# spacemeshos/go-spacemesh

Hardware: AMD Instinct MI355X
Metric: post_labels_per_sec (higher is better)
Workload: dtype u32; 1 GPU; init-mainnet-scryptN8192-4units-256GiB-sink; step_labels=2097152, scrypt_n=8192, num_units=4, labels_per_unit=4294967296, parallelism=index-range shards x1, RCCL nonce min-reduce, vrf_nonce_found=True

## Files before the change

go-spacemesh_amd/csrc/kernels.hip:

```cpp
#include <hip/hip_runtime.h>

#include <cstdlib>
#include <cstring>

#include "kernel_args.h"
#include "post_common.h"

#define POSTE_THREADS 256

#if defined(POSTE_NT) && POSTE_NT
typedef uint32_t poste_v4u __attribute__((ext_vector_type(4)));
#define VSTORE(p, v)                                                           \
  do {                                                                         \
    uint4 _t = (v);                                                            \
    __builtin_nontemporal_store(*(poste_v4u *)&_t, (poste_v4u *)(p));          \
  } while (0)
#define VLOAD(p)                                                               \
  ({                                                                           \
    poste_v4u _r = __builtin_nontemporal_load((const poste_v4u *)(p));         \
    *(uint4 *)&_r;                                                             \
  })
#else
#define VSTORE(p, v) (*(p) = (v))
#define VLOAD(p) (*(p))
#endif

__constant__ uint32_t c_sha_k[64] = {
    0x428a2f98, 0x71374491, 0xb5c0fbcf, 0xe9b5dba5, 0x3956c25b, 0x59f111f1,
    0x923f82a4, 0xab1c5ed5, 0xd807aa98, 0x12835b01, 0x243185be, 0x550c7dc3,
    0x72be5d74, 0x80deb1fe, 0x9bdc06a7, 0xc19bf174, 0xe49b69c1, 0xefbe4786,
    0x0fc19dc6, 0x240ca1cc, 0x2de92c6f, 0x4a7484aa, 0x5cb0a9dc, 0x76f988da,
    0x983e5152, 0xa831c66d, 0xb00327c8, 0xbf597fc7, 0xc6e00bf3, 0xd5a79147,
    0x06ca6351, 0x14292967, 0x27b70a85, 0x2e1b2138, 0x4d2c6dfc, 0x53380d13,
    0x650a7354, 0x766a0abb, 0x81c2c92e, 0x92722c85, 0xa2bfe8a1, 0xa81a664b,
    0xc24b8b70, 0xc76c51a3, 0xd192e819, 0xd6990624, 0xf40e3585, 0x106aa070,
    0x19a4c116, 0x1e376c08, 0x2748774c, 0x34b0bcb5, 0x391c0cb3, 0x4ed8aa4a,
    0x5b9cca4f, 0x682e6ff3, 0x748f82ee, 0x78a5636f, 0x84c87814, 0x8cc70208,
    0x90befffa, 0xa4506ceb, 0xbef9a3f7, 0xc67178f2};

__device__ __forceinline__ uint32_t ror32(uint32_t x, int n) {
  return __builtin_rotateright32(x, n);
}

__device__ void sha_compress(uint32_t h[8], const uint32_t m[16]) {
  uint32_t w[16];
#pragma unroll
  for (int i = 0; i < 16; i++) w[i] = m[i];
  uint32_t a = h[0], b = h[1], c = h[2], d = h[3];
  uint32_t e = h[4], f = h[5], g = h[6], hh = h[7];
#pragma unroll
  for (int t = 0; t < 64; t++) {
    uint32_t wt;
    if (t < 16) {
      wt = w[t];
    } else {
      uint32_t a15 = w[(t - 15) & 15], a2 = w[(t - 2) & 15];
      wt = w[t & 15] += (ror32(a15, 7) ^ ror32(a15, 18) ^ (a15 >> 3)) +
                        w[(t - 7) & 15] +
                        (ror32(a2, 17) ^ ror32(a2, 19) ^ (a2 >> 10));
    }
    uint32_t t1 = hh + (ror32(e, 6) ^ ror32(e, 11) ^ ror32(e, 25)) +
                  ((e & f) ^ (~e & g)) + c_sha_k[t] + wt;
    uint32_t t2 = (ror32(a, 2) ^ ror32(a, 13) ^ ror32(a, 22)) +
                  ((a & b) ^ (a & c) ^ (b & c));
    hh = g; g = f; f = e; e = d + t1;
    d = c; c = b; b = a; a = t1 + t2;
  }
  h[0] += a; h[1] += b; h[2] += c; h[3] += d;
  h[4] += e; h[5] += f; h[6] += g; h[7] += hh;
}

__device__ __forceinline__ void sha_init(uint32_t h[8]) {
  h[0] = 0x6a09e667; h[1] = 0xbb67ae85; h[2] = 0x3c6ef372; h[3] = 0xa54ff53a;
  h[4] = 0x510e527f; h[5] = 0x9b05688c; h[6] = 0x1f83d9ab; h[7] = 0x5be0cd19;
}


#define SWZ(v, pat)                                                            \
  ((uint32_t)__builtin_amdgcn_mov_dpp((int)(v), (pat), 0xf, 0xf, true))
#define QROT1 0x39
#define QROT2 0x4E
#define QROT3 0x93
#define QBCAST0 0x00

__device__ __forceinline__ void salsa8_z(uint32_t &A, uint32_t &B,
                                         uint32_t &C, uint32_t &D) {
  uint32_t a = A, b = B, c = C, d = D;
#pragma unroll
  for (int i = 0; i < 4; i++) {
    b ^= __builtin_rotateleft32(a + d, 7);
    c ^= __builtin_rotateleft32(b + a, 9);
    d ^= __builtin_rotateleft32(c + b, 13);
    a ^= __builtin_rotateleft32(d + c, 18);
    uint32_t y1 = SWZ(d, QROT1);
    uint32_t y2 = SWZ(c, QROT2);
    uint32_t y3 = SWZ(b, QROT3);
    y1 ^= __builtin_rotateleft32(a + y3, 7);
    y2 ^= __builtin_rotateleft32(y1 + a, 9);
    y3 ^= __builtin_rotateleft32(y2 + y1, 13);
    a ^= __builtin_rotateleft32(y3 + y2, 18);
    d = SWZ(y1, QROT3);
    c = SWZ(y2, QROT2);
    b = SWZ(y3, QROT1);
  }
  A += a; B += b; C += c; D += d;
}

__device__ __forceinline__ void blockmix_z(uint32_t X0[4], uint32_t X1[4]) {
  uint32_t t0 = X0[0] ^ X1[0], t1 = X0[1] ^ X1[1], t2 = X0[2] ^ X1[2],
           t3 = X0[3] ^ X1[3];
  salsa8_z(t0, t1, t2, t3);
  X0[0] = t0; X0[1] = t1; X0[2] = t2; X0[3] = t3;
  t0 ^= X1[0]; t1 ^= X1[1]; t2 ^= X1[2]; t3 ^= X1[3];
  salsa8_z(t0, t1, t2, t3);
  X1[0] = t0; X1[1] = t1; X1[2] = t2; X1[3] = t3;
}

__device__ __forceinline__ void canon_to_z(const uint32_t x[16], uint32_t sub,
                                           uint32_t z[4]) {
  uint32_t s0 = sub == 0 ? x[0] : sub == 1 ? x[5] : sub == 2 ? x[10] : x[15];
  uint32_t s1 = sub == 0 ? x[4] : sub == 1 ? x[9] : sub == 2 ? x[14] : x[3];
  uint32_t s2 = sub == 0 ? x[8] : sub == 1 ? x[13] : sub == 2 ? x[2] : x[7];
  uint32_t s3 = sub == 0 ? x[12] : sub == 1 ? x[1] : sub == 2 ? x[6] : x[11];
  z[0] = s0; z[1] = s1; z[2] = s2; z[3] = s3;
}

__device__ __forceinline__ void z_to_msg_be(const uint32_t z[4],
                                            uint32_t m[16]) {
#pragma unroll
  for (int v = 0; v < 4; v++) {
    m[(4 * v + 0) & 15] = __builtin_bswap32(SWZ(z[v], 0x00));
    m[(4 * v + 5) & 15] = __builtin_bswap32(SWZ(z[v], 0x55));
    m[(4 * v + 10) & 15] = __builtin_bswap32(SWZ(z[v], 0xAA));
    m[(4 * v + 15) & 15] = __builtin_bswap32(SWZ(z[v], 0xFF));
  }
}


__device__ __forceinline__ void hmac_outer(const uint32_t ho[8],
                                           const uint32_t inner[8],
                                           uint32_t out[8]) {
  uint32_t h[8], m[16];
#pragma unroll
  for (int i = 0; i < 8; i++) h[i] = ho[i];
#pragma unroll
  for (int i = 0; i < 8; i++) m[i] = inner[i];
  m[8] = 0x80000000u;
#pragma unroll
  for (int i = 9; i < 15; i++) m[i] = 0;
  m[15] = (64 + 32) * 8;
  sha_compress(h, m);
#pragma unroll
  for (int i = 0; i < 8; i++) out[i] = h[i];
}


__device__ __forceinline__ void hmac_states_for(const uint32_t *cw,
                                                unsigned long long index,
                                                uint32_t hi[8],
                                                uint32_t ho[8]) {
  uint32_t pw_be[10], m[16];
#pragma unroll
  for (int i = 0; i < 8; i++) pw_be[i] = __builtin_bswap32(cw[i]);
  pw_be[8] = __builtin_bswap32((uint32_t)index);
  pw_be[9] = __builtin_bswap32((uint32_t)(index >> 32));
  sha_init(hi);
#pragma unroll
  for (int i = 0; i < 10; i++) m[i] = pw_be[i] ^ 0x36363636u;
#pragma unroll
  for (int i = 10; i < 16; i++) m[i] = 0x36363636u;
  sha_compress(hi, m);
  sha_init(ho);
#pragma unroll
  for (int i = 0; i < 10; i++) m[i] = pw_be[i] ^ 0x5c5c5c5cu;
#pragma unroll
  for (int i = 10; i < 16; i++) m[i] = 0x5c5c5c5cu;
  sha_compress(ho, m);
}

__global__ void __launch_bounds__(POSTE_THREADS)
post_label_prologue_kernel(LabelKernelArgs a) {
  const unsigned long long lane =
      (unsigned long long)blockIdx.x * blockDim.x + threadIdx.x;
  const unsigned long long group = lane >> 2;
  const unsigned long long gstride =
      ((unsigned long long)gridDim.x * blockDim.x) >> 2;
  const uint32_t sub = (uint32_t)(lane & 3);
  uint4 *X = (uint4 *)a.xbuf;

  for (unsigned long long task = group; task < a.count;
       task += gstride) {
    const unsigned long long index = a.indices ? a.indices[task]
                                               : a.start + task;
    const uint32_t *cw = a.commit_ids
                             ? a.commitments + 8ull * a.commit_ids[task]
                             : a.commitment_le;
    uint32_t hi[8], ho[8], m[16];
    hmac_states_for(cw, index, hi, ho);
    uint32_t Z0[4], Z1[4];
    for (uint32_t half = 0; half < 2; half++) {
      uint32_t cblk[16];
#pragma unroll
      for (uint32_t q = 0; q < 2; q++) {
        const uint32_t blk = half * 2 + q + 1;
        uint32_t h[8];
#pragma unroll
        for (int i = 0; i < 8; i++) h[i] = hi[i];
        m[0] = blk;
        m[1] = 0x80000000u;
#pragma unroll
        for (int i = 2; i < 15; i++) m[i] = 0;
        m[15] = (64 + 4) * 8;
        sha_compress(h, m);
        uint32_t d[8];
        hmac_outer(ho, h, d);
#pragma unroll
        for (int k = 0; k < 8; k++)
          cblk[8 * q + k] = __builtin_bswap32(d[k]);
      }
      canon_to_z(cblk, sub, half == 0 ? Z0 : Z1);
    }
    uint4 *p = X + task * 8ull;
    p[sub] = make_uint4(Z0[0], Z0[1], Z0[2], Z0[3]);
    p[sub + 4] = make_uint4(Z1[0], Z1[1], Z1[2], Z1[3]);
  }
}

__global__ void __launch_bounds__(POSTE_THREADS, 8)
post_label_romix_gap_kernel(LabelKernelArgs a) {
  const unsigned long long lane =
      (unsigned long long)blockIdx.x * blockDim.x + threadIdx.x;
  const unsigned long long group = lane >> 2;
  const uint32_t sub = (uint32_t)(lane & 3);
  const uint32_t n = a.scrypt_n;
  const uint32_t mask = n - 1;
  const uint32_t gmask = (1u << a.gap_shift) - 1u;
  uint4 *V = (uint4 *)a.scratch;
  uint4 *X = (uint4 *)a.xbuf;

  for (unsigned long long task = group; task < a.count;
       task += a.scratch_lanes) {
    uint32_t Z0[4], Z1[4];
    {
      uint4 *p = X + task * 8ull;
      uint4 v0 = p[sub], v1 = p[sub + 4];
      Z0[0] = v0.x; Z0[1] = v0.y; Z0[2] = v0.z; Z0[3] = v0.w;
      Z1[0] = v1.x; Z1[1] = v1.y; Z1[2] = v1.z; Z1[3] = v1.w;
    }
    {
      unsigned long long base = group * 8ull + sub;
      const unsigned long long stride = a.scratch_lanes * 8ull;
      for (uint32_t j = 0; j < n; j++) {
        if ((j & gmask) == 0) {
          uint4 *p = V + base;
          VSTORE(p, make_uint4(Z0[0], Z0[1], Z0[2], Z0[3]));
          VSTORE(p + 4, make_uint4(Z1[0], Z1[1], Z1[2], Z1[3]));
          base += stride;
        }
        blockmix_z(Z0, Z1);
      }
    }
    for (uint32_t i = 0; i < n; i++) {
      uint32_t j = SWZ(Z1[0], QBCAST0) & mask;
      const uint32_t r = j & gmask;
      const uint4 *p =
          V + ((unsigned long long)(j >> a.gap_shift) * a.scratch_lanes +
               group) * 8ull + sub;
      uint32_t Y0[4], Y1[4];
      {
        uint4 v0 = VLOAD(p), v1 = VLOAD(p + 4);
        Y0[0] = v0.x; Y0[1] = v0.y; Y0[2] = v0.z; Y0[3] = v0.w;
        Y1[0] = v1.x; Y1[1] = v1.y; Y1[2] = v1.z; Y1[3] = v1.w;
      }
      for (uint32_t t = 0; t < r; t++) blockmix_z(Y0, Y1);
#pragma unroll
      for (int k = 0; k < 4; k++) {
        Z0[k] ^= Y0[k];
        Z1[k] ^= Y1[k];
      }
      blockmix_z(Z0, Z1);
    }
    {
      uint4 *p = X + task * 8ull;
      p[sub] = make_uint4(Z0[0], Z0[1], Z0[2], Z0[3]);
      p[sub + 4] = make_uint4(Z1[0], Z1[1], Z1[2], Z1[3]);
    }
  }
}

#define POSTE_U24 0xffffffu

__device__ __forceinline__ const uint4 *vblock(const uint4 *qbase, uint32_t j,
                                               uint32_t stride16) {
  return qbase + (unsigned long long)j * stride16;
}

#define XOR3(a, b, c) ((uint32_t)__builtin_amdgcn_bitop3_b32((a), (b), (c), 0x96))

__device__ __forceinline__ void blockmix_xor_z(uint32_t X0[4], uint32_t X1[4],
                                               const uint4 v0,
                                               const uint4 v1) {
  X1[0] ^= v1.x; X1[1] ^= v1.y; X1[2] ^= v1.z; X1[3] ^= v1.w;
  uint32_t t0 = XOR3(X0[0], v0.x, X1[0]), t1 = XOR3(X0[1], v0.y, X1[1]),
           t2 = XOR3(X0[2], v0.z, X1[2]), t3 = XOR3(X0[3], v0.w, X1[3]);
  salsa8_z(t0, t1, t2, t3);
  X0[0] = t0; X0[1] = t1; X0[2] = t2; X0[3] = t3;
  t0 ^= X1[0]; t1 ^= X1[1]; t2 ^= X1[2]; t3 ^= X1[3];
  salsa8_z(t0, t1, t2, t3);
  X1[0] = t0; X1[1] = t1; X1[2] = t2; X1[3] = t3;
}

__global__ void __launch_bounds__(POSTE_THREADS, 8)
post_label_romix_kernel(LabelKernelArgs a) {
  const unsigned long long lane =
      (unsigned long long)blockIdx.x * blockDim.x + threadIdx.x;
  const unsigned long long group = lane >> 2;
  const uint32_t sub = (uint32_t)(lane & 3);
  const uint32_t n = a.scrypt_n;
  const uint32_t mask = (n - 1) & POSTE_U24;
  const uint32_t stride16 = ((uint32_t)a.scratch_lanes * 8u) & POSTE_U24;
  uint4 *const qbase = (uint4 *)a.scratch + (group * 8ull + sub);
  uint4 *X = (uint4 *)a.xbuf;

  for (unsigned long long task = group; task < a.count;
       task += a.scratch_lanes) {
    uint32_t Z0[4], Z1[4];
    {
      uint4 *p = X + task * 8ull;
      uint4 v0 = p[sub], v1 = p[sub + 4];
      Z0[0] = v0.x; Z0[1] = v0.y; Z0[2] = v0.z; Z0[3] = v0.w;
      Z1[0] = v1.x; Z1[1] = v1.y; Z1[2] = v1.z; Z1[3] = v1.w;
    }
    {
      uint4 *p = qbase;
      for (uint32_t j = 0; j < n; j++) {
        VSTORE(p, make_uint4(Z0[0], Z0[1], Z0[2], Z0[3]));
        VSTORE(p + 4, make_uint4(Z1[0], Z1[1], Z1[2], Z1[3]));
        p += stride16;
        blockmix_z(Z0, Z1);
      }
    }
    for (uint32_t i = 0; i < n; i++) {
      const uint32_t j = SWZ(Z1[0], QBCAST0) & mask;
      const uint4 *p = vblock(qbase, j, stride16);
      const uint4 v0 = VLOAD(p), v1 = VLOAD(p + 4);
      blockmix_xor_z(Z0, Z1, v0, v1);
    }
    {
      uint4 *p = X + task * 8ull;
      p[sub] = make_uint4(Z0[0], Z0[1], Z0[2], Z0[3]);
      p[sub + 4] = make_uint4(Z1[0], Z1[1], Z1[2], Z1[3]);
    }
  }
}

__global__ void __launch_bounds__(POSTE_THREADS, 8)
post_label_romix_fill_kernel(RomixPhaseArgs a) {
  const unsigned long long lane =
      (unsigned long long)blockIdx.x * blockDim.x + threadIdx.x;
  const unsigned long long task = lane >> 2;
  const uint32_t sub = (uint32_t)(lane & 3);
  if (task >= a.count || task >= a.slot_count) return;
  const uint32_t n = a.scrypt_n;
  const uint32_t stride16 = ((uint32_t)a.scratch_lanes * 8u) & POSTE_U24;
  uint4 *p = (uint4 *)a.scratch + ((a.slot_base + task) * 8ull + sub);
  uint4 *x = (uint4 *)a.xbuf + task * 8ull;

  uint32_t Z0[4], Z1[4];
  {
    uint4 v0 = x[sub], v1 = x[sub + 4];
    Z0[0] = v0.x; Z0[1] = v0.y; Z0[2] = v0.z; Z0[3] = v0.w;
    Z1[0] = v1.x; Z1[1] = v1.y; Z1[2] = v1.z; Z1[3] = v1.w;
  }
  for (uint32_t j = 0; j < n; j++) {
    VSTORE(p, make_uint4(Z0[0], Z0[1], Z0[2], Z0[3]));
    VSTORE(p + 4, make_uint4(Z1[0], Z1[1], Z1[2], Z1[3]));
    p += stride16;
    blockmix_z(Z0, Z1);
  }
  x[sub] = make_uint4(Z0[0], Z0[1], Z0[2], Z0[3]);
  x[sub + 4] = make_uint4(Z1[0], Z1[1], Z1[2], Z1[3]);
}

__global__ void __launch_bounds__(POSTE_THREADS, 8)
post_label_romix_mix_kernel(RomixPhaseArgs a) {
  const unsigned long long lane =
      (unsigned long long)blockIdx.x * blockDim.x + threadIdx.x;
  const unsigned long long task = lane >> 2;
  const uint32_t sub = (uint32_t)(lane & 3);
  if (task >= a.count || task >= a.slot_count) return;
  const uint32_t n = a.scrypt_n;
  const uint32_t mask = (n - 1) & POSTE_U24;
  const uint32_t stride16 = ((uint32_t)a.scratch_lanes * 8u) & POSTE_U24;
  const uint4 *const qbase =
      (const uint4 *)a.scratch + ((a.slot_base + task) * 8ull + sub);
  uint4 *x = (uint4 *)a.xbuf + task * 8ull;

  uint32_t Z0[4], Z1[4];
  {
    uint4 v0 = x[sub], v1 = x[sub + 4];
    Z0[0] = v0.x; Z0[1] = v0.y; Z0[2] = v0.z; Z0[3] = v0.w;
    Z1[0] = v1.x; Z1[1] = v1.y; Z1[2] = v1.z; Z1[3] = v1.w;
  }
  for (uint32_t i = 0; i < n; i++) {
    const uint32_t j = SWZ(Z1[0], QBCAST0) & mask;
    const uint4 *p = vblock(qbase, j, stride16);
    const uint4 v0 = VLOAD(p), v1 = VLOAD(p + 4);
    blockmix_xor_z(Z0, Z1, v0, v1);
  }
  x[sub] = make_uint4(Z0[0], Z0[1], Z0[2], Z0[3]);
  x[sub + 4] = make_uint4(Z1[0], Z1[1], Z1[2], Z1[3]);
}

__global__ void __launch_bounds__(POSTE_THREADS)
post_label_tail_kernel(LabelKernelArgs a) {
  const unsigned long long lane =
      (unsigned long long)blockIdx.x * blockDim.x + threadIdx.x;
  const unsigned long long group = lane >> 2;
  const unsigned long long gstride =
      ((unsigned long long)gridDim.x * blockDim.x) >> 2;
  const uint32_t sub = (uint32_t)(lane & 3);
  uint4 *X = (uint4 *)a.xbuf;

  uint32_t min_lab[8];
  unsigned long long min_idx = 0;
  int min_found = 0;

  for (unsigned long long task = group; task < a.count;
       task += gstride) {
    const unsigned long long index = a.indices ? a.indices[task]
                                               : a.start + task;
    const uint32_t *cw = a.commit_ids
                             ? a.commitments + 8ull * a.commit_ids[task]
                             : a.commitment_le;
    uint32_t hi[8], ho[8], m[16];
    hmac_states_for(cw, index, hi, ho);
    uint32_t Z0[4], Z1[4];
    {
      uint4 *p = X + task * 8ull;
      uint4 v0 = p[sub], v1 = p[sub + 4];
      Z0[0] = v0.x; Z0[1] = v0.y; Z0[2] = v0.z; Z0[3] = v0.w;
      Z1[0] = v1.x; Z1[1] = v1.y; Z1[2] = v1.z; Z1[3] = v1.w;
    }
    uint32_t h[8];
#pragma unroll
    for (int i = 0; i < 8; i++) h[i] = hi[i];
    z_to_msg_be(Z0, m);
    sha_compress(h, m);
    z_to_msg_be(Z1, m);
    sha_compress(h, m);
    m[0] = 1;
    m[1] = 0x80000000u;
#pragma unroll
    for (int i = 2; i < 15; i++) m[i] = 0;
    m[15] = (64 + 128 + 4) * 8;
    sha_compress(h, m);
    uint32_t lab_be[8];
    hmac_outer(ho, h, lab_be);

    if (a.out && sub == 0) {
      if (a.out_full) {
        uint4 *o = (uint4 *)(a.out + task * 32ull);
        o[0] = make_uint4(__builtin_bswap32(lab_be[0]),
                          __builtin_bswap32(lab_be[1]),
                          __builtin_bswap32(lab_be[2]),
                          __builtin_bswap32(lab_be[3]));
        o[1] = make_uint4(__builtin_bswap32(lab_be[4]),
                          __builtin_bswap32(lab_be[5]),
                          __builtin_bswap32(lab_be[6]),
                          __builtin_bswap32(lab_be[7]));
      } else {
        *(uint4 *)(a.out + task * 16ull) =
            make_uint4(__builtin_bswap32(lab_be[0]),
                       __builtin_bswap32(lab_be[1]),
                       __builtin_bswap32(lab_be[2]),
                       __builtin_bswap32(lab_be[3]));
      }
    }

    if (a.has_difficulty && sub == 0) {
      bool below_diff = false, below_min = false;
#pragma unroll
      for (int k = 0; k < 8; k++) {
        if (lab_be[k] != a.difficulty_be[k]) {
          below_diff = lab_be[k] < a.difficulty_be[k];
          break;
        }
      }
      if (below_diff) {
        if (!min_found) {
          below_min = true;
        } else {
          below_min = false;
#pragma unroll
          for (int k = 0; k < 8; k++) {
            if (lab_be[k] != min_lab[k]) {
              below_min = lab_be[k] < min_lab[k];
              break;
            }
          }
        }
        if (below_min) {
          min_found = 1;
          min_idx = index;
#pragma unroll
          for (int k = 0; k < 8; k++) min_lab[k] = lab_be[k];
        }
      }
    }
  }

  if (a.has_difficulty) {
    __shared__ uint32_t s_lab[POSTE_THREADS][8];
    __shared__ unsigned long long s_idx[POSTE_THREADS];
    __shared__ uint8_t s_found[POSTE_THREADS];
    s_found[threadIdx.x] = (uint8_t)min_found;
    if (min_found) {
      s_idx[threadIdx.x] = min_idx;
#pragma unroll
      for (int k = 0; k < 8; k++) s_lab[threadIdx.x][k] = min_lab[k];
    }
    __syncthreads();
    if (threadIdx.x == 0) {
      int best = -1;
      for (int t = 0; t < POSTE_THREADS; t++) {
        if (!s_found[t]) continue;
        if (best < 0) {
          best = t;
          continue;
        }
        int cmp = 0;
        for (int k = 0; k < 8 && cmp == 0; k++) {
          if (s_lab[t][k] < s_lab[best][k]) cmp = -1;
          else if (s_lab[t][k] > s_lab[best][k]) cmp = 1;
        }
        if (cmp < 0 || (cmp == 0 && s_idx[t] < s_idx[best])) best = t;
      }
      if (best >= 0) {
        unsigned int slot = atomicAdd(a.cand_count, 1u);
        if (slot < a.cand_cap) {
          a.cand[slot].index = s_idx[best];
          for (int k = 0; k < 8; k++)
            a.cand[slot].label_be[k] = s_lab[best][k];
        }
      }
    }
  }
}

__global__ void __launch_bounds__(POSTE_THREADS)
post_label_audit_tail_kernel(AuditKernelArgs aa) {
  const LabelKernelArgs &a = aa.label;
  const unsigned long long lane =
      (unsigned long long)blockIdx.x * blockDim.x + threadIdx.x;
  const unsigned long long group = lane >> 2;
  const unsigned long long gstride =
      ((unsigned long long)gridDim.x * blockDim.x) >> 2;
  const uint32_t sub = (uint32_t)(lane & 3);
  const uint4 *X = (const uint4 *)a.xbuf;

  for (unsigned long long task = group; task < a.count;
       task += gstride) {
    const unsigned long long index = a.indices ? a.indices[task]
                                               : a.start + task;
    const uint32_t *cw = a.commit_ids
                             ? a.commitments + 8ull * a.commit_ids[task]
                             : a.commitment_le;
    uint32_t hi[8], ho[8], m[16];
    hmac_states_for(cw, index, hi, ho);
    uint32_t Z0[4], Z1[4];
    {
      const uint4 *p = X + task * 8ull;
      uint4 v0 = p[sub], v1 = p[sub + 4];
      Z0[0] = v0.x; Z0[1] = v0.y; Z0[2] = v0.z; Z0[3] = v0.w;
      Z1[0] = v1.x; Z1[1] = v1.y; Z1[2] = v1.z; Z1[3] = v1.w;
    }
    uint32_t h[8];
#pragma unroll
    for (int i = 0; i < 8; i++) h[i] = hi[i];
    z_to_msg_be(Z0, m);
    sha_compress(h, m);
    z_to_msg_be(Z1, m);
    sha_compress(h, m);
    m[0] = 1;
    m[1] = 0x80000000u;
#pragma unroll
    for (int i = 2; i < 15; i++) m[i] = 0;
    m[15] = (64 + 128 + 4) * 8;
    sha_compress(h, m);
    uint32_t lab_be[8];
    hmac_outer(ho, h, lab_be);

    if (sub == 0) {
      const uint4 want = aa.expected[task];
      const uint4 got = make_uint4(__builtin_bswap32(lab_be[0]),
                                   __builtin_bswap32(lab_be[1]),
                                   __builtin_bswap32(lab_be[2]),
                                   __builtin_bswap32(lab_be[3]));
      if (got.x != want.x || got.y != want.y || got.z != want.z ||
          got.w != want.w) {
        const unsigned int slot = atomicAdd(aa.count, 1u);
        PostAuditMismatch *o = aa.mismatch + slot;
        o->index = index;
        o->label[0] = got.x;
        o->label[1] = got.y;
        o->label[2] = got.z;
        o->label[3] = got.w;
      }
    }
  }
}


__global__ void __launch_bounds__(POSTE_THREADS)
post_scan_kernel(ScanKernelArgs a) {
#if defined(POSTE_SCAN_GLOBAL_TT)
  const uint32_t *TE_LO = a.te;
  const uint32_t *TE_HI = a.te;
  const uint8_t *sSbox = a.sbox;
#elif defined(POSTE_SCAN_SPLIT_TT)
  extern __shared__ uint32_t lds[];
  uint32_t *TE_LO = lds;
  const uint32_t *TE_HI = a.te;
  uint8_t *sSbox = (uint8_t *)(lds + 512);
  for (uint32_t i = threadIdx.x; i < 512; i += blockDim.x) TE_LO[i] = a.te[i];
  for (uint32_t i = threadIdx.x; i < 256; i += blockDim.x)
    sSbox[i] = a.sbox[i];
  __syncthreads();
#else
  extern __shared__ uint32_t lds[];
  uint32_t *sTe = lds;
  uint8_t *sSbox = (uint8_t *)(sTe + 1024);
  uint32_t *TE_LO = sTe, *TE_HI = sTe;

  for (uint32_t i = threadIdx.x; i < 1024; i += blockDim.x) sTe[i] = a.te[i];
  for (uint32_t i = threadIdx.x; i < 256; i += blockDim.x)
    sSbox[i] = a.sbox[i];
  __syncthreads();
#endif

  const unsigned long long stride =
      (unsigned long long)gridDim.x * blockDim.x;
#ifndef POSTE_SCAN_ILP
#define POSTE_SCAN_ILP 2
#endif
  constexpr int L = POSTE_SCAN_ILP;
  const unsigned long long span = stride * L;
  for (unsigned long long t0 =
           (unsigned long long)blockIdx.x * blockDim.x + threadIdx.x;
       t0 < a.count; t0 += span) {
    uint32_t p[L][4];
    unsigned long long ts[L];
#pragma unroll
    for (int u = 0; u < L; u++) {
      unsigned long long t = t0 + (unsigned long long)u * stride;
      ts[u] = t < a.count ? t : t0;
      uint4 lraw = a.labels[ts[u]];
      p[u][0] = __builtin_bswap32(lraw.x);
      p[u][1] = __builtin_bswap32(lraw.y);
      p[u][2] = __builtin_bswap32(lraw.z);
      p[u][3] = __builtin_bswap32(lraw.w);
    }
    const int live = (int)((a.count - t0 + stride - 1) / stride) < L
                         ? (int)((a.count - t0 + stride - 1) / stride)
                         : L;
    for (uint32_t c = 0; c < a.n_ciphers; c++) {
      const uint32_t *rk = a.rk + c * 44;
      uint32_t w[L][4];
#pragma unroll
      for (int u = 0; u < L; u++)
#pragma unroll
        for (int k = 0; k < 4; k++) w[u][k] = p[u][k] ^ rk[k];
#pragma unroll
      for (int r = 1; r < 10; r++) {
#pragma unroll
        for (int u = 0; u < L; u++) {
          uint32_t n0 = TE_LO[w[u][0] >> 24] ^
                        TE_LO[256 + ((w[u][1] >> 16) & 0xff)] ^
                        TE_HI[512 + ((w[u][2] >> 8) & 0xff)] ^
                        TE_HI[768 + (w[u][3] & 0xff)] ^ rk[4 * r];
          uint32_t n1 = TE_LO[w[u][1] >> 24] ^
                        TE_LO[256 + ((w[u][2] >> 16) & 0xff)] ^
                        TE_HI[512 + ((w[u][3] >> 8) & 0xff)] ^
                        TE_HI[768 + (w[u][0] & 0xff)] ^ rk[4 * r + 1];
          uint32_t n2 = TE_LO[w[u][2] >> 24] ^
                        TE_LO[256 + ((w[u][3] >> 16) & 0xff)] ^
                        TE_HI[512 + ((w[u][0] >> 8) & 0xff)] ^
                        TE_HI[768 + (w[u][1] & 0xff)] ^ rk[4 * r + 2];
          uint32_t n3 = TE_LO[w[u][3] >> 24] ^
                        TE_LO[256 + ((w[u][0] >> 16) & 0xff)] ^
                        TE_HI[512 + ((w[u][1] >> 8) & 0xff)] ^
                        TE_HI[768 + (w[u][2] & 0xff)] ^ rk[4 * r + 3];
          w[u][0] = n0; w[u][1] = n1; w[u][2] = n2; w[u][3] = n3;
        }
      }
#pragma unroll
      for (int u = 0; u < L; u++) {
        if (u >= live) break;
        uint32_t f0 = (((uint32_t)sSbox[w[u][0] >> 24] << 24) |
                       ((uint32_t)sSbox[(w[u][1] >> 16) & 0xff] << 16) |
                       ((uint32_t)sSbox[(w[u][2] >> 8) & 0xff] << 8) |
                       sSbox[w[u][3] & 0xff]) ^ rk[40];
        uint32_t f1 = (((uint32_t)sSbox[w[u][1] >> 24] << 24) |
                       ((uint32_t)sSbox[(w[u][2] >> 16) & 0xff] << 16) |
                       ((uint32_t)sSbox[(w[u][3] >> 8) & 0xff] << 8) |
                       sSbox[w[u][0] & 0xff]) ^ rk[41];
        uint32_t f2 = (((uint32_t)sSbox[w[u][2] >> 24] << 24) |
                       ((uint32_t)sSbox[(w[u][3] >> 16) & 0xff] << 16) |
                       ((uint32_t)sSbox[(w[u][0] >> 8) & 0xff] << 8) |
                       sSbox[w[u][1] & 0xff]) ^ rk[42];
        uint32_t f3 = (((uint32_t)sSbox[w[u][3] >> 24] << 24) |
                       ((uint32_t)sSbox[(w[u][0] >> 16) & 0xff] << 16) |
                       ((uint32_t)sSbox[(w[u][1] >> 8) & 0xff] << 8) |
                       sSbox[w[u][2] & 0xff]) ^ rk[43];
        unsigned long long v0 =
            __builtin_bswap64(((unsigned long long)f0 << 32) | f1);
        unsigned long long v1 =
            __builtin_bswap64(((unsigned long long)f2 << 32) | f3);
        if (v0 < a.difficulty) {
          unsigned int s = atomicAdd(a.hit_count, 1u);
          if (s < a.hit_cap) {
            a.hits[s].index = a.index_base + ts[u];
            a.hits[s].nonce = c * POSTE_NONCES_PER_AES;
          }
        }
        if (v1 < a.difficulty) {
          unsigned int s = atomicAdd(a.hit_count, 1u);
          if (s < a.hit_cap) {
            a.hits[s].index = a.index_base + ts[u];
            a.hits[s].nonce = c * POSTE_NONCES_PER_AES + 1;
          }
        }
      }
    }
  }
}

#define ROR8(x) __builtin_amdgcn_alignbit((x), (x), 8)
#define ROR16(x) __builtin_amdgcn_alignbit((x), (x), 16)
#define ROR24(x) __builtin_amdgcn_alignbit((x), (x), 24)

template <int THREADS_, bool BATCHG>
__global__ void __launch_bounds__(THREADS_)
post_scan_bankrep_kernel(ScanKernelArgs a) {
  extern __shared__ uint32_t sTe[];
  for (uint32_t i = threadIdx.x; i < 8192; i += blockDim.x)
// ... 343 lines not shown
#pragma unroll
  for (int i = 0; i < 3; i++) {
    if ((uint32_t)i < rest) {
      const uint4 l = src[4 * full + i];
      m[4 * i] = __builtin_bswap32(l.x);
      m[4 * i + 1] = __builtin_bswap32(l.y);
      m[4 * i + 2] = __builtin_bswap32(l.z);
      m[4 * i + 3] = __builtin_bswap32(l.w);
    }
  }
#pragma unroll
  for (int i = 0; i < 4; i++)
    if ((uint32_t)i == rest) m[4 * i] = 0x80000000u;
  m[15] = n * 128;
  sha_compress(h, m);
  a.digests[page] =
      make_uint4(__builtin_bswap32(h[0]), __builtin_bswap32(h[1]),
                 __builtin_bswap32(h[2]), __builtin_bswap32(h[3]));
}

__device__ __forceinline__ void seal_msg_label(uint32_t *m, const uint4 l) {
  m[0] = __builtin_bswap32(l.x);
  m[1] = __builtin_bswap32(l.y);
  m[2] = __builtin_bswap32(l.z);
  m[3] = __builtin_bswap32(l.w);
}

__global__ void __launch_bounds__(POSTE_SEAL_THREADS)
post_seal_stream_kernel(SealStreamArgs a) {
  const unsigned long long end = a.g0 + a.count;
  const unsigned long long p0 = a.g0 / POSTE_SEAL_PAGE_LABELS;
  const unsigned long long lanes = (end - 1) / POSTE_SEAL_PAGE_LABELS - p0 + 1;
  const unsigned long long lane =
      (unsigned long long)blockIdx.x * blockDim.x + threadIdx.x;
  if (lane >= lanes) return;
  const unsigned long long page_lo = (p0 + lane) * POSTE_SEAL_PAGE_LABELS;
  const unsigned long long page_hi = page_lo + POSTE_SEAL_PAGE_LABELS;
  const unsigned long long lo = page_lo > a.g0 ? page_lo : a.g0;
  const unsigned long long hi = page_hi < end ? page_hi : end;
  const uint32_t n_seg = (uint32_t)(hi - lo);
  const uint32_t before = (uint32_t)(lo - page_lo);
  const bool closes = hi == page_hi || hi == a.stream_end;
  const uint4 *src = a.labels + (lo - a.g0);

  uint32_t h[8], m[16];
  uint4 buf[3];
  uint32_t r = 0;
  if (before) {
    const uint4 *c = (const uint4 *)a.carry_in;
    const uint4 h0 = c[0], h1 = c[1];
    h[0] = h0.x; h[1] = h0.y; h[2] = h0.z; h[3] = h0.w;
    h[4] = h1.x; h[5] = h1.y; h[6] = h1.z; h[7] = h1.w;
    r = before % 4;
#pragma unroll
    for (int i = 0; i < 3; i++) buf[i] = c[3 + i];
  } else {
    sha_init(h);
#pragma unroll
    for (int i = 0; i < 3; i++) buf[i] = make_uint4(0, 0, 0, 0);
  }
  const uint32_t msg = r + n_seg;
  const uint32_t full = msg / 4, rest = msg % 4;

  uint4 q[4];
  if (full) {
#pragma unroll
    for (int i = 0; i < 4; i++) {
      if ((uint32_t)i < r) {
        if (i < 3) q[i] = buf[i];
      } else {
        q[i] = src[i - r];
      }
    }
  }
  for (uint32_t b = 0; b < full; b++) {
#pragma unroll
    for (int i = 0; i < 4; i++) seal_msg_label(m + 4 * i, q[i]);
    if (b + 1 < full) {
      const uint4 *nx = src + (4 * (b + 1) - r);
#pragma unroll
      for (int i = 0; i < 4; i++) q[i] = nx[i];
    }
    sha_compress(h, m);
  }
  uint4 t[3];
#pragma unroll
  for (int i = 0; i < 3; i++) {
    t[i] = make_uint4(0, 0, 0, 0);
    if ((uint32_t)i < rest)
      t[i] = (full == 0 && (uint32_t)i < r) ? buf[i] : src[4 * full + i - r];
  }
  if (!closes) {
    uint4 *c = (uint4 *)a.carry_out;
    c[0] = make_uint4(h[0], h[1], h[2], h[3]);
    c[1] = make_uint4(h[4], h[5], h[6], h[7]);
    c[2] = make_uint4(before + n_seg, 0, 0, 0);
#pragma unroll
    for (int i = 0; i < 3; i++) c[3 + i] = t[i];
    return;
  }
#pragma unroll
  for (int i = 0; i < 16; i++) m[i] = 0;
#pragma unroll
  for (int i = 0; i < 3; i++)
    if ((uint32_t)i < rest) seal_msg_label(m + 4 * i, t[i]);
#pragma unroll
  for (int i = 0; i < 4; i++)
    if ((uint32_t)i == rest) m[4 * i] = 0x80000000u;
  m[15] = (before + n_seg) * 128;
  sha_compress(h, m);
  a.digests[lane] =
      make_uint4(__builtin_bswap32(h[0]), __builtin_bswap32(h[1]),
                 __builtin_bswap32(h[2]), __builtin_bswap32(h[3]));
}

extern "C" {

hipError_t poste_launch_seal_stream_kernel(const SealStreamArgs *args,
                                           hipStream_t stream) {
  if (!args->labels || !args->digests || !args->carry_in ||
      !args->carry_out || args->carry_in == args->carry_out ||
      args->count == 0 || args->g0 + args->count < args->g0 ||
      args->g0 + args->count > args->stream_end)
    return hipErrorInvalidValue;
  const uint64_t lanes = (args->g0 + args->count - 1) / POSTE_SEAL_PAGE_LABELS -
                         args->g0 / POSTE_SEAL_PAGE_LABELS + 1;
  hipLaunchKernelGGL(
      post_seal_stream_kernel,
      dim3((uint32_t)((lanes + POSTE_SEAL_THREADS - 1) / POSTE_SEAL_THREADS)),
      dim3(POSTE_SEAL_THREADS), 0, stream, *args);
  return hipGetLastError();
}

hipError_t poste_launch_seal_kernel(const SealKernelArgs *args,
                                    hipStream_t stream) {
  if (!args->labels || !args->digests || args->count == 0)
    return hipErrorInvalidValue;
  const uint64_t pages =
      (args->count + POSTE_SEAL_PAGE_LABELS - 1) / POSTE_SEAL_PAGE_LABELS;
  hipLaunchKernelGGL(
      post_seal_kernel,
      dim3((uint32_t)((pages + POSTE_SEAL_THREADS - 1) / POSTE_SEAL_THREADS)),
      dim3(POSTE_SEAL_THREADS), 0, stream, *args);
  return hipGetLastError();
}

int poste_label_romix_lean_ok(uint32_t scrypt_n, uint32_t gap_shift,
                              uint64_t scratch_lanes) {
  return gap_shift == 0 && scrypt_n <= (1u << 24) &&
         scratch_lanes < (1ull << 21) &&
         (uint64_t)scrypt_n * scratch_lanes < (1ull << 32);
}

static void launch_label_prologue_romix(const LabelKernelArgs *args,
                                        uint32_t blocks, hipStream_t stream) {
  hipLaunchKernelGGL(post_label_prologue_kernel, dim3(blocks),
                     dim3(POSTE_THREADS), 0, stream, *args);
  if (poste_label_romix_lean_ok(args->scrypt_n, args->gap_shift,
                                args->scratch_lanes)) {
    hipLaunchKernelGGL(post_label_romix_kernel, dim3(blocks),
                       dim3(POSTE_THREADS), 0, stream, *args);
  } else {
    hipLaunchKernelGGL(post_label_romix_gap_kernel, dim3(blocks),
                       dim3(POSTE_THREADS), 0, stream, *args);
  }
}

hipError_t poste_launch_label_kernel(const LabelKernelArgs *args,
                                     uint32_t blocks, hipStream_t stream) {
  launch_label_prologue_romix(args, blocks, stream);
  hipLaunchKernelGGL(post_label_tail_kernel, dim3(blocks),
                     dim3(POSTE_THREADS), 0, stream, *args);
  return hipGetLastError();
}

hipError_t poste_launch_label_prologue(const LabelKernelArgs *args,
                                       uint32_t blocks, hipStream_t stream) {
  hipLaunchKernelGGL(post_label_prologue_kernel, dim3(blocks),
                     dim3(POSTE_THREADS), 0, stream, *args);
  return hipGetLastError();
}

hipError_t poste_launch_label_tail(const LabelKernelArgs *args,
                                   uint32_t blocks, hipStream_t stream) {
  hipLaunchKernelGGL(post_label_tail_kernel, dim3(blocks),
                     dim3(POSTE_THREADS), 0, stream, *args);
  return hipGetLastError();
}

static bool romix_phase_ok(const RomixPhaseArgs *a) {
  return a->count >= 1 && a->count <= a->slot_count &&
         a->slot_base + a->slot_count <= a->scratch_lanes &&
         poste_label_romix_lean_ok(a->scrypt_n, 0, a->scratch_lanes);
}

hipError_t poste_launch_romix_fill(const RomixPhaseArgs *args,
                                   hipStream_t stream) {
  if (!romix_phase_ok(args)) return hipErrorInvalidValue;
  const uint32_t quads = POSTE_THREADS / 4;
  hipLaunchKernelGGL(post_label_romix_fill_kernel,
                     dim3((uint32_t)((args->count + quads - 1) / quads)),
                     dim3(POSTE_THREADS), 0, stream, *args);
  return hipGetLastError();
}

hipError_t poste_launch_romix_mix(const RomixPhaseArgs *args,
                                  hipStream_t stream) {
  if (!romix_phase_ok(args)) return hipErrorInvalidValue;
  const uint32_t quads = POSTE_THREADS / 4;
  hipLaunchKernelGGL(post_label_romix_mix_kernel,
                     dim3((uint32_t)((args->count + quads - 1) / quads)),
                     dim3(POSTE_THREADS), 0, stream, *args);
  return hipGetLastError();
}

hipError_t poste_launch_label_audit(const AuditKernelArgs *args,
                                    uint32_t blocks, hipStream_t stream) {
  launch_label_prologue_romix(&args->label, blocks, stream);
  hipLaunchKernelGGL(post_label_audit_tail_kernel, dim3(blocks),
                     dim3(POSTE_THREADS), 0, stream, *args);
  return hipGetLastError();
}

hipError_t poste_launch_verify_pred_kernel(const VerifyPredArgs *args,
                                           uint32_t blocks,
                                           hipStream_t stream) {
  size_t lds = 1024 * 4 + 256;
  hipLaunchKernelGGL(post_verify_pred_kernel, dim3(blocks),
                     dim3(POSTE_THREADS), lds, stream, *args);
  return hipGetLastError();
}

uint64_t poste_label_resident_slots(uint32_t gap_shift) {
  const void *kern =
      gap_shift == 0
          ? reinterpret_cast<const void *>(post_label_romix_kernel)
          : reinterpret_cast<const void *>(post_label_romix_gap_kernel);
  int blocks_per_cu = 0;
  if (hipOccupancyMaxActiveBlocksPerMultiprocessor(&blocks_per_cu, kern,
                                                   POSTE_THREADS, 0) !=
          hipSuccess ||
      blocks_per_cu <= 0)
    blocks_per_cu = 2;
  hipDeviceProp_t prop;
  int dev = 0;
  (void)hipGetDevice(&dev);
  int cus = 256;
  if (hipGetDeviceProperties(&prop, dev) == hipSuccess)
    cus = prop.multiProcessorCount;
  return (uint64_t)blocks_per_cu * cus * (POSTE_THREADS / 4);
}

static uint32_t scan_block_cap(uint32_t variant_cap) {
  const char *e = getenv("POST_SCAN_MAX_BLOCKS");
  if (!e) return variant_cap;
  long v = strtol(e, nullptr, 10);
  return v >= 1 && v < (long)variant_cap ? (uint32_t)v : variant_cap;
}

hipError_t poste_launch_scan_kernel(const ScanKernelArgs *args,
                                    uint32_t blocks, hipStream_t stream) {
  const uint32_t cap = scan_block_cap(8192);
  if (blocks > cap) blocks = cap;
  const char *e = getenv("POST_SCAN_MODE");
  const char *m = e ? e : "tt4";
  if (strcmp(m, "shared") == 0) {
    size_t lds = 1024 * 4 + 256;
    hipLaunchKernelGGL(post_scan_kernel, dim3(blocks), dim3(POSTE_THREADS),
                       lds, stream, *args);
    return hipGetLastError();
  }
  if (strcmp(m, "tt4") == 0) {
    static bool attr_ok = [] {
      return hipFuncSetAttribute(
                 (const void *)post_scan_tt4_kernel,
                 hipFuncAttributeMaxDynamicSharedMemorySize,
                 32768 * 4) == hipSuccess;
    }();
    if (attr_ok) {
      uint32_t b4 = (uint32_t)((args->count + 1023) / 1024);
      const uint32_t cap4 = scan_block_cap(2048);
      if (b4 > cap4) b4 = cap4;
      if (b4 == 0) b4 = 1;
      hipLaunchKernelGGL(post_scan_tt4_kernel, dim3(b4), dim3(1024),
                         32768 * 4, stream, *args);
      return hipGetLastError();
    }
    m = "bankrep";
  }
  const bool bg = strstr(m, "bg") != nullptr;
  const bool wide = strstr(m, "512") != nullptr;
  size_t lds = 8192 * 4;
  if (wide) {
    uint32_t b5 = (uint32_t)((args->count + 511) / 512);
    const uint32_t cap5 = scan_block_cap(4096);
    if (b5 > cap5) b5 = cap5;
    if (b5 == 0) b5 = 1;
    if (bg)
      hipLaunchKernelGGL((post_scan_bankrep_kernel<512, true>), dim3(b5),
                         dim3(512), lds, stream, *args);
    else
      hipLaunchKernelGGL((post_scan_bankrep_kernel<512, false>), dim3(b5),
                         dim3(512), lds, stream, *args);
  } else if (bg) {
    hipLaunchKernelGGL((post_scan_bankrep_kernel<POSTE_THREADS, true>),
                       dim3(blocks), dim3(POSTE_THREADS), lds, stream,
                       *args);
  } else {
    hipLaunchKernelGGL((post_scan_bankrep_kernel<POSTE_THREADS, false>),
                       dim3(blocks), dim3(POSTE_THREADS), lds, stream,
                       *args);
  }
  return hipGetLastError();
}
}
```

Baseline: 2.157 million labels/s.

## Run PBKDF2 prologue and tail with one thread per label instead of quads

The prologue, tail and audit-tail kernels previously had four lanes each redundantly compute the full HMAC-SHA256 work for a label, with each lane keeping only its quarter. Now one thread handles a whole label, writing and reading all eight uint4 chunks in the quad-interleaved layout the romix kernels expect. The grid for these SHA kernels is capped to the blocks actually needed. This removes 4x redundant SHA work, at the cost of higher per-thread register pressure and strided uint4 memory accesses.

```diff
diff --git a/go-spacemesh_amd/csrc/kernels.hip b/go-spacemesh_amd/csrc/kernels.hip
--- a/go-spacemesh_amd/csrc/kernels.hip
+++ b/go-spacemesh_amd/csrc/kernels.hip
@@ -116,26 +116,6 @@
   X1[0] = t0; X1[1] = t1; X1[2] = t2; X1[3] = t3;
 }
 
-__device__ __forceinline__ void canon_to_z(const uint32_t x[16], uint32_t sub,
-                                           uint32_t z[4]) {
-  uint32_t s0 = sub == 0 ? x[0] : sub == 1 ? x[5] : sub == 2 ? x[10] : x[15];
-  uint32_t s1 = sub == 0 ? x[4] : sub == 1 ? x[9] : sub == 2 ? x[14] : x[3];
-  uint32_t s2 = sub == 0 ? x[8] : sub == 1 ? x[13] : sub == 2 ? x[2] : x[7];
-  uint32_t s3 = sub == 0 ? x[12] : sub == 1 ? x[1] : sub == 2 ? x[6] : x[11];
-  z[0] = s0; z[1] = s1; z[2] = s2; z[3] = s3;
-}
-
-__device__ __forceinline__ void z_to_msg_be(const uint32_t z[4],
-                                            uint32_t m[16]) {
-#pragma unroll
-  for (int v = 0; v < 4; v++) {
-    m[(4 * v + 0) & 15] = __builtin_bswap32(SWZ(z[v], 0x00));
-    m[(4 * v + 5) & 15] = __builtin_bswap32(SWZ(z[v], 0x55));
-    m[(4 * v + 10) & 15] = __builtin_bswap32(SWZ(z[v], 0xAA));
-    m[(4 * v + 15) & 15] = __builtin_bswap32(SWZ(z[v], 0xFF));
-  }
-}
-
 
 __device__ __forceinline__ void hmac_outer(const uint32_t ho[8],
                                            const uint32_t inner[8],
@@ -178,18 +158,36 @@
   sha_compress(ho, m);
 }
 
+
+__device__ __forceinline__ void canon_to_chunks(const uint32_t x[16],
+                                                uint4 *p) {
+#pragma unroll
+  for (int c = 0; c < 4; c++)
+    p[c] = make_uint4(x[(5 * c) & 15], x[(4 + 5 * c) & 15],
+                      x[(8 + 5 * c) & 15], x[(12 + 5 * c) & 15]);
+}
+
+__device__ __forceinline__ void chunks_to_msg_be(const uint4 *p,
+                                                 uint32_t m[16]) {
+#pragma unroll
+  for (int c = 0; c < 4; c++) {
+    const uint4 v = p[c];
+    m[(5 * c) & 15] = __builtin_bswap32(v.x);
+    m[(4 + 5 * c) & 15] = __builtin_bswap32(v.y);
+    m[(8 + 5 * c) & 15] = __builtin_bswap32(v.z);
+    m[(12 + 5 * c) & 15] = __builtin_bswap32(v.w);
+  }
+}
+
 __global__ void __launch_bounds__(POSTE_THREADS)
 post_label_prologue_kernel(LabelKernelArgs a) {
   const unsigned long long lane =
       (unsigned long long)blockIdx.x * blockDim.x + threadIdx.x;
-  const unsigned long long group = lane >> 2;
   const unsigned long long gstride =
-      ((unsigned long long)gridDim.x * blockDim.x) >> 2;
-  const uint32_t sub = (uint32_t)(lane & 3);
+      (unsigned long long)gridDim.x * blockDim.x;
   uint4 *X = (uint4 *)a.xbuf;
 
-  for (unsigned long long task = group; task < a.count;
-       task += gstride) {
+  for (unsigned long long task = lane; task < a.count; task += gstride) {
     const unsigned long long index = a.indices ? a.indices[task]
                                                : a.start + task;
     const uint32_t *cw = a.commit_ids
@@ -197,7 +195,7 @@
                              : a.commitment_le;
     uint32_t hi[8], ho[8], m[16];
     hmac_states_for(cw, index, hi, ho);
-    uint32_t Z0[4], Z1[4];
+    uint4 *p = X + task * 8ull;
     for (uint32_t half = 0; half < 2; half++) {
       uint32_t cblk[16];
 #pragma unroll
@@ -218,11 +216,8 @@
         for (int k = 0; k < 8; k++)
           cblk[8 * q + k] = __builtin_bswap32(d[k]);
       }
-      canon_to_z(cblk, sub, half == 0 ? Z0 : Z1);
-    }
-    uint4 *p = X + task * 8ull;
-    p[sub] = make_uint4(Z0[0], Z0[1], Z0[2], Z0[3]);
-    p[sub + 4] = make_uint4(Z1[0], Z1[1], Z1[2], Z1[3]);
+      canon_to_chunks(cblk, p + 4 * half);
+    }
   }
 }
 
@@ -416,18 +411,15 @@
 post_label_tail_kernel(LabelKernelArgs a) {
   const unsigned long long lane =
       (unsigned long long)blockIdx.x * blockDim.x + threadIdx.x;
-  const unsigned long long group = lane >> 2;
   const unsigned long long gstride =
-      ((unsigned long long)gridDim.x * blockDim.x) >> 2;
-  const uint32_t sub = (uint32_t)(lane & 3);
+      (unsigned long long)gridDim.x * blockDim.x;
   uint4 *X = (uint4 *)a.xbuf;
 
   uint32_t min_lab[8];
   unsigned long long min_idx = 0;
   int min_found = 0;
 
-  for (unsigned long long task = group; task < a.count;
-       task += gstride) {
+  for (unsigned long long task = lane; task < a.count; task += gstride) {
     const unsigned long long index = a.indices ? a.indices[task]
                                                : a.start + task;
     const uint32_t *cw = a.commit_ids
@@ -435,19 +427,13 @@
                              : a.commitment_le;
     uint32_t hi[8], ho[8], m[16];
     hmac_states_for(cw, index, hi, ho);
-    uint32_t Z0[4], Z1[4];
-    {
-      uint4 *p = X + task * 8ull;
-      uint4 v0 = p[sub], v1 = p[sub + 4];
-      Z0[0] = v0.x; Z0[1] = v0.y; Z0[2] = v0.z; Z0[3] = v0.w;
-      Z1[0] = v1.x; Z1[1] = v1.y; Z1[2] = v1.z; Z1[3] = v1.w;
-    }
+    const uint4 *p = X + task * 8ull;
     uint32_t h[8];
 #pragma unroll
     for (int i = 0; i < 8; i++) h[i] = hi[i];
-    z_to_msg_be(Z0, m);
+    chunks_to_msg_be(p, m);
     sha_compress(h, m);
-    z_to_msg_be(Z1, m);
+    chunks_to_msg_be(p + 4, m);
     sha_compress(h, m);
     m[0] = 1;
     m[1] = 0x80000000u;
@@ -458,7 +444,7 @@
     uint32_t lab_be[8];
     hmac_outer(ho, h, lab_be);
 
-    if (a.out && sub == 0) {
+    if (a.out) {
       if (a.out_full) {
         uint4 *o = (uint4 *)(a.out + task * 32ull);
         o[0] = make_uint4(__builtin_bswap32(lab_be[0]),
@@ -478,7 +464,7 @@
       }
     }
 
-    if (a.has_difficulty && sub == 0) {
+    if (a.has_difficulty) {
       bool below_diff = false, below_min = false;
 #pragma unroll
       for (int k = 0; k < 8; k++) {
@@ -553,14 +539,11 @@
   const LabelKernelArgs &a = aa.label;
   const unsigned long long lane =
       (unsigned long long)blockIdx.x * blockDim.x + threadIdx.x;
-  const unsigned long long group = lane >> 2;
   const unsigned long long gstride =
-      ((unsigned long long)gridDim.x * blockDim.x) >> 2;
-  const uint32_t sub = (uint32_t)(lane & 3);
+      (unsigned long long)gridDim.x * blockDim.x;
   const uint4 *X = (const uint4 *)a.xbuf;
 
-  for (unsigned long long task = group; task < a.count;
-       task += gstride) {
+  for (unsigned long long task = lane; task < a.count; task += gstride) {
     const unsigned long long index = a.indices ? a.indices[task]
                                                : a.start + task;
     const uint32_t *cw = a.commit_ids
@@ -568,19 +551,13 @@
                              : a.commitment_le;
     uint32_t hi[8], ho[8], m[16];
     hmac_states_for(cw, index, hi, ho);
-    uint32_t Z0[4], Z1[4];
-    {
-      const uint4 *p = X + task * 8ull;
-      uint4 v0 = p[sub], v1 = p[sub + 4];
-      Z0[0] = v0.x; Z0[1] = v0.y; Z0[2] = v0.z; Z0[3] = v0.w;
-      Z1[0] = v1.x; Z1[1] = v1.y; Z1[2] = v1.z; Z1[3] = v1.w;
-    }
+    const uint4 *p = X + task * 8ull;
     uint32_t h[8];
 #pragma unroll
     for (int i = 0; i < 8; i++) h[i] = hi[i];
-    z_to_msg_be(Z0, m);
+    chunks_to_msg_be(p, m);
     sha_compress(h, m);
-    z_to_msg_be(Z1, m);
+    chunks_to_msg_be(p + 4, m);
     sha_compress(h, m);
     m[0] = 1;
     m[1] = 0x80000000u;
@@ -591,7 +568,7 @@
     uint32_t lab_be[8];
     hmac_outer(ho, h, lab_be);
 
-    if (sub == 0) {
+    {
       const uint4 want = aa.expected[task];
       const uint4 got = make_uint4(__builtin_bswap32(lab_be[0]),
                                    __builtin_bswap32(lab_be[1]),
@@ -1241,10 +1218,17 @@
          (uint64_t)scrypt_n * scratch_lanes < (1ull << 32);
 }
 
+static uint32_t sha_blocks(const LabelKernelArgs *args, uint32_t blocks) {
+  const uint64_t need = (args->count + POSTE_THREADS - 1) / POSTE_THREADS;
+  const uint64_t g = need < blocks ? need : blocks;
+  return g ? (uint32_t)g : 1u;
+}
+
 static void launch_label_prologue_romix(const LabelKernelArgs *args,
                                         uint32_t blocks, hipStream_t stream) {
-  hipLaunchKernelGGL(post_label_prologue_kernel, dim3(blocks),
-                     dim3(POSTE_THREADS), 0, stream, *args);
+  hipLaunchKernelGGL(post_label_prologue_kernel,
+                     dim3(sha_blocks(args, blocks)), dim3(POSTE_THREADS), 0,
+                     stream, *args);
   if (poste_label_romix_lean_ok(args->scrypt_n, args->gap_shift,
                                 args->scratch_lanes)) {
     hipLaunchKernelGGL(post_label_romix_kernel, dim3(blocks),
@@ -1258,21 +1242,22 @@
 hipError_t poste_launch_label_kernel(const LabelKernelArgs *args,
                                      uint32_t blocks, hipStream_t stream) {
   launch_label_prologue_romix(args, blocks, stream);
-  hipLaunchKernelGGL(post_label_tail_kernel, dim3(blocks),
+  hipLaunchKernelGGL(post_label_tail_kernel, dim3(sha_blocks(args, blocks)),
                      dim3(POSTE_THREADS), 0, stream, *args);
   return hipGetLastError();
 }
 
 hipError_t poste_launch_label_prologue(const LabelKernelArgs *args,
                                        uint32_t blocks, hipStream_t stream) {
-  hipLaunchKernelGGL(post_label_prologue_kernel, dim3(blocks),
-                     dim3(POSTE_THREADS), 0, stream, *args);
+  hipLaunchKernelGGL(post_label_prologue_kernel,
+                     dim3(sha_blocks(args, blocks)), dim3(POSTE_THREADS), 0,
+                     stream, *args);
   return hipGetLastError();
 }
 
 hipError_t poste_launch_label_tail(const LabelKernelArgs *args,
                                    uint32_t blocks, hipStream_t stream) {
-  hipLaunchKernelGGL(post_label_tail_kernel, dim3(blocks),
+  hipLaunchKernelGGL(post_label_tail_kernel, dim3(sha_blocks(args, blocks)),
                      dim3(POSTE_THREADS), 0, stream, *args);
   return hipGetLastError();
 }
@@ -1306,7 +1291,8 @@
 hipError_t poste_launch_label_audit(const AuditKernelArgs *args,
                                     uint32_t blocks, hipStream_t stream) {
   launch_label_prologue_romix(&args->label, blocks, stream);
-  hipLaunchKernelGGL(post_label_audit_tail_kernel, dim3(blocks),
+  hipLaunchKernelGGL(post_label_audit_tail_kernel,
+                     dim3(sha_blocks(&args->label, blocks)),
                      dim3(POSTE_THREADS), 0, stream, *args);
   return hipGetLastError();
 }
```

Measured after the change: 2.181 million labels/s (median of 6 runs). +1.1%, better.
